# bwittmann/transoar

Hardware: AMD Instinct MI355X
Metric: training-step CT volumes/s, 160x160x256 Focused-Decoder (higher is better)
Workload: dtype bf16

## Files before the change

include/transoar_conv3d.h:

```cpp
#ifndef TRANSOAR_CONV3D_H
#define TRANSOAR_CONV3D_H

#include <stddef.h>
#include <stdint.h>

#ifdef __cplusplus
extern "C" {
#endif

enum {
  TRANSOAR_CONV_OK = 0,
  TRANSOAR_CONV_ERR_NULL = -1,
  TRANSOAR_CONV_ERR_DIM = -2,
  TRANSOAR_CONV_ERR_CHANNELS = -3
};

int transoar_conv3d_k3_forward(const void* x, const void* wk, const float* bias, void* y,
                               int N, int D, int H, int W, int Cin, int Cout, int stride,
                               int dilated_input, void* hip_stream);

int transoar_conv3d_k3_wgrad(const void* gyT, const void* xT3, float* dw, int N, int D, int H,
                             int W, int Cin, int Do, int Ho, int Wo, int Cout, int stride_dh,
                             void* hip_stream);

int transoar_conv3d_k3_forward_c1(const void* x, const void* wk, const float* bias, void* y, int N, int D, int H,
                                  int W, int Cout, void* hip_stream);

int transoar_conv3d_k3_stat_rows(int N, int D, int H, int W, int Cin, int Cout, int stride);
int transoar_conv3d_k3_forward_stats(const void* x, const void* wk, const float* bias, void* y, float* stat_part,
                                     int N, int D, int H, int W, int Cin, int Cout, void* hip_stream);

int transoar_conv3d_c1_forward(const void* x, const float* w, void* y, int N, int D, int H,
                               int W, int Cout, void* hip_stream);

int transoar_conv3d_k3_wgrad_lds(const void* x, const void* dy, float* partial, int n_wg, int N, int D,
                                 int H, int W, int Cin, int Cout, int ci0, int ci_n, int co0, int co_n,
                                 void* hip_stream);
int transoar_conv3d_k3_wgrad_tr(const void* x, const void* dy, float* partial, int n_wg, int N, int D,
                                 int H, int W, int Cin, int Cout, int ci0, int ci_n, int co0, int co_n,
                                 void* hip_stream);

int transoar_conv3d_c1_wgrad(const void* x, const void* dy, float* partial, int n_partial, int N, int D,
                             int H, int W, int Cout, void* hip_stream);
int transoar_conv3d_c1_wgrad_tr(const void* x, const void* dy, float* partial, int n_partial, int N, int D,
                                int H, int W, int Cout, void* hip_stream);

int transoar_layout_bf16(const void* in, void* out, int N, long V, int C, int to_channels_first,
                         void* hip_stream);

int transoar_conv3d_abi_version(void);

#ifdef __cplusplus
}
#endif
#endif
```

include/transoar_instnorm.h:

```cpp
#ifndef TRANSOAR_INSTNORM_H
#define TRANSOAR_INSTNORM_H

#ifdef __cplusplus
extern "C" {
#endif

enum {
  TRANSOAR_IN_OK = 0,
  TRANSOAR_IN_ERR_NULL = -1,
  TRANSOAR_IN_ERR_DIM = -2,
  TRANSOAR_IN_ERR_CHANNELS = -3
};

int transoar_instnorm_relu_forward(const void* x, const float* gamma, const float* beta, void* y,
                                   double* stats_ws, float* mean_rstd, int N, long V, int C,
                                   float eps, int relu, void* hip_stream);

int transoar_instnorm_relu_forward_parts(const void* x, const float* gamma, const float* beta, void* y,
                                         const float* stat_part, int rows_per_sample, double* stats_ws,
                                         float* mean_rstd, int N, long V, int C, float eps, int relu,
                                         void* hip_stream);

int transoar_instnorm_relu_backward(const void* x, const void* dy, const float* gamma,
                                    const float* beta, const float* mean_rstd, void* dx,
                                    double* red_ws, float* dparams, int N, long V, int C, int relu,
                                    void* hip_stream);

int transoar_instnorm_abi_version(void);

#ifdef __cplusplus
}
#endif
#endif
```

transoar_amd/backbone.py:

```python
import os

import torch
from torch import nn

from . import instnorm
from .conv3d import Conv3dK3, to_ncdhw
from .position_encoding import PositionEmbeddingLearned3D, PositionEmbeddingSine3D
from .swin_encoder import ConvPatchMerging, EncoderSwinBlock, PatchMerging
from .refine_block import DecoderDefAttnBlock
from .token_linear import token_linear


class EncoderCnnBlock(nn.Module):

    def __init__(self, in_channels, out_channels, kernel_size, stride, padding=1, bias=False,
                 affine=True, eps=1e-05):
        super().__init__()
        kernel_size, stride = tuple(kernel_size), tuple(stride)
        self._block = nn.Sequential(
            Conv3dK3(in_channels, out_channels, kernel_size, stride=stride, padding=padding, bias=bias),
            nn.InstanceNorm3d(out_channels, affine=affine, eps=eps),
            nn.ReLU(inplace=True),
            Conv3dK3(out_channels, out_channels, kernel_size, stride=1, padding=padding, bias=bias),
            nn.InstanceNorm3d(out_channels, affine=affine, eps=eps),
            nn.ReLU(inplace=True),
        )
        self._affine = affine

    fused_norm = True

    def _norm_relu(self, x, norm, part=None):
        if (EncoderCnnBlock.fused_norm and self._affine and x.dtype == torch.bfloat16
                and instnorm.supported(x, norm.num_features)):
            return instnorm.instance_norm_relu(x, norm.weight, norm.bias, norm.eps, relu=True, part=part)
        return torch.relu_(norm(x))

    def _conv_norm_relu(self, conv, norm, x):
        if (EncoderCnnBlock.fused_norm and self._affine and isinstance(conv, Conv3dK3) and norm.num_features <= 32):
            y, part = conv.forward_with_stats(x)
            if part is not None and not (y.dtype == torch.bfloat16 and instnorm.supported(y, norm.num_features)):
                part = None
            return self._norm_relu(y, norm, part)
        return self._norm_relu(conv(x), norm)

    def forward(self, x):
        if not x.is_cuda:
            return self._block(x)
        blk = self._block
        x = self._conv_norm_relu(blk[0], blk[1], x)
        return self._conv_norm_relu(blk[3], blk[4], x)


class Encoder(nn.Module):
    def __init__(self, config, debug=False):
        super().__init__()
        self._debug = debug
        self._stages = nn.ModuleList()
        cin, cout = config["in_channels"], config["start_channels"]
        swin = bool(config["use_encoder_attn"])
        depths = list(config["depths"])
        dpr = [float(v) for v in torch.linspace(0, config["drop_path_rate"], sum(depths))]
        merge = ConvPatchMerging if config["conv_merging"] else PatchMerging
        for stage_id, (kernel, stride) in enumerate(zip(config["conv_kernels"], config["strides"])):
            if swin and stage_id > 1:
                k = stage_id - 2
                stage = EncoderSwinBlock(
                    dim=cin, depth=depths[k], num_heads=config["num_heads"][k], window_size=config["window_size"],
                    mlp_ratio=config["mlp_ratio"], qkv_bias=config["qkv_bias"], qk_scale=config["qk_scale"],
                    drop=config["drop_rate"], attn_drop=config["attn_drop_rate"],
                    drop_path=dpr[sum(depths[:k]):sum(depths[:k + 1])], downsample=merge)
            else:
                stage = EncoderCnnBlock(cin, cout, kernel, stride)
# ... 134 lines not shown
```

transoar_amd/conv3d.py:

```python
import ctypes
import os

import torch
import torch.nn.functional as F
from torch import nn

from . import _native
from . import rows as _rows
from . import conv_gemm as _cg

_PKG = os.path.dirname(os.path.abspath(__file__))
_LIB_PATH = os.path.join(_PKG, "libtransoar_conv3d.so")
ABI_VERSION = 5


def _load():
    if not os.path.exists(_LIB_PATH):
        raise _native.NativeLibraryError("%s is not built (python transoar_amd/_build.py)" % _LIB_PATH)
    lib = ctypes.CDLL(_LIB_PATH)
    i, p = ctypes.c_int, ctypes.c_void_p
    lib.transoar_conv3d_k3_forward.restype = i
    lib.transoar_conv3d_k3_forward.argtypes = [p, p, p, p] + [i] * 8 + [p]
    lib.transoar_conv3d_k3_wgrad.restype = i
    lib.transoar_conv3d_k3_wgrad.argtypes = [p, p, p] + [i] * 10 + [p]
    lib.transoar_conv3d_k3_wgrad_lds.restype = i
    lib.transoar_conv3d_k3_wgrad_lds.argtypes = [p, p, p, i] + [i] * 10 + [p]
    lib.transoar_conv3d_k3_wgrad_tr.restype = i
    lib.transoar_conv3d_k3_wgrad_tr.argtypes = [p, p, p, i] + [i] * 10 + [p]
    lib.transoar_conv3d_c1_wgrad.restype = i
    lib.transoar_conv3d_c1_wgrad.argtypes = [p, p, p, i] + [i] * 5 + [p]
    lib.transoar_conv3d_c1_wgrad_tr.restype = i
    lib.transoar_conv3d_c1_wgrad_tr.argtypes = [p, p, p, i] + [i] * 5 + [p]
    lib.transoar_conv3d_k3_stat_rows.restype = i
    lib.transoar_conv3d_k3_stat_rows.argtypes = [i] * 7
    lib.transoar_conv3d_k3_forward_stats.restype = i
    lib.transoar_conv3d_k3_forward_stats.argtypes = [p, p, p, p, p] + [i] * 6 + [p]
    lib.transoar_conv3d_k3_forward_c1.restype = i
    lib.transoar_conv3d_k3_forward_c1.argtypes = [p, p, p, p] + [i] * 5 + [p]
    lib.transoar_conv3d_c1_forward.restype = i
    lib.transoar_conv3d_c1_forward.argtypes = [p, p, p] + [i] * 5 + [p]
    lib.transoar_layout_bf16.restype = i
    lib.transoar_layout_bf16.argtypes = [p, p, i, ctypes.c_long, i, i, p]
    lib.transoar_conv3d_abi_version.restype = i
    if lib.transoar_conv3d_abi_version() != ABI_VERSION:
        raise _native.NativeLibraryError("%s: ABI mismatch, rebuild" % _LIB_PATH)
    return lib


lib = _load()
CL3D = torch.channels_last_3d


def _check(rc, what):
    if rc != 0:
        raise RuntimeError("%s failed with code %d" % (what, rc))


def _stream():
    return torch.cuda.current_stream().cuda_stream


class _Relayout(torch.autograd.Function):

# ... 197 lines not shown
                wk, wkt = packs
            elif weight.requires_grad or x.requires_grad:
                wk, wkt = _cg.pack_both(weight)
            else:
                wk = _cg.pack_fwd(weight)
            y = _cg.conv_forward(xb, wk, bias.float() if bias is not None else None, stride)
        else:
            y = conv3d_k3_forward(xb, _pack_taps(weight), bias.float() if bias is not None else None, stride)
        ctx.save_for_backward(xb, weight, wkt)
        ctx.stride, ctx.has_bias = stride, bias is not None
        return (y, None) if want_stats else y

    @staticmethod
    def backward(ctx, gy, _gpart=None):
        xb, weight, wkt = ctx.saved_tensors
        gyb = _as_ndhwc(gy)
        gx = gw = gb = None
        need_x, need_w = ctx.needs_input_grad[0], ctx.needs_input_grad[1]
        ci, co = xb.shape[1], weight.shape[0]
        if need_x and _use_gemm(ci, co, ctx.stride):
            gx = _cg.conv_dgrad(gyb, wkt if wkt is not None else _cg.pack_dgrad(weight), ctx.stride, tuple(xb.shape[2:]))
        elif need_x:
            wt = weight.flip(2, 3, 4).permute(2, 3, 4, 1, 0).reshape(27, weight.shape[1], weight.shape[0])
            gx = conv3d_k3_forward(gyb, wt.to(torch.bfloat16).contiguous(), None, 1, dilated_input=ctx.stride == 2)
        if need_w:
            rows = gyb.numel() // gyb.shape[1]
            if ctx.stride == 1 and c1_wgrad_supported(xb, gyb):
                gw = conv3d_c1_wgrad(xb, gyb)
            elif ctx.stride == 1 and lds_wgrad_supported(xb, gyb) and (max(ci, co) <= 32 or rows >= (1 << 21)):
                gw = conv3d_k3_wgrad_lds(xb, gyb)
            elif ci % 8 == 0 and co % 8 == 0:
                gw = _cg.conv_wgrad(xb, gyb, ctx.stride)
            else:
                gw = conv3d_k3_wgrad(xb, gyb, ctx.stride)
            gw = gw.to(weight.dtype)
        if ctx.has_bias and ctx.needs_input_grad[2]:
            g2 = gyb.permute(0, 2, 3, 4, 1).reshape(-1, gyb.shape[1])
            gb = _rows.colsum_any(g2) if g2.is_contiguous() else gyb.float().sum(dim=(0, 2, 3, 4))
        return gx, gw, gb, None, None, None


def _use_gemm(cin, cout, stride):
    return cin >= 8 and cin % 8 == 0 and cout % 8 == 0 and (stride == 2 or cin > 24 or cout > 32)


def hip_conv_supported(x, conv):
    return (x.is_cuda and x.dtype == torch.bfloat16 and conv.kernel_size == (3, 3, 3) and conv.padding == (1, 1, 1)
            and conv.stride in ((1, 1, 1), (2, 2, 2)) and conv.dilation == (1, 1, 1) and conv.groups == 1
            and (conv.in_channels % 8 == 0
                 or (conv.in_channels == 1 and conv.stride == (1, 1, 1) and conv.out_channels <= 64))
            and conv.out_channels % 8 == 0 and (x.shape[-1] // conv.stride[0]) % 8 == 0
            and (conv.stride == (1, 1, 1) or all(s % 2 == 0 for s in x.shape[2:])))


class Conv3dK3(nn.Conv3d):
    enabled = True
    min_voxels = 0
    ndhwc_everywhere = os.environ.get("TRANSOAR_NDHWC_ALL", "1") == "1"
    _packs, _packs_version = None, -1

    def uses_gemm(self):
        return self.kernel_size == (3, 3, 3) and _use_gemm(self.in_channels, self.out_channels, self.stride[0])

    def forward(self, x):
# ... 22 lines not shown
```

transoar_amd/csrc/conv3d.hip:

```cpp
#include <hip/hip_runtime.h>
#include <algorithm>
#include <cstdlib>
#include <stdint.h>

#include "../../include/transoar_conv3d.h"

namespace transoar {

using bf16x8 = __attribute__((ext_vector_type(8))) __bf16;
using f32x16 = __attribute__((ext_vector_type(16))) float;
using u32x4c = __attribute__((ext_vector_type(4))) unsigned int;
using u32x2c = __attribute__((ext_vector_type(2))) unsigned int;

__device__ __forceinline__ unsigned short f2bf(float f) {
  return __builtin_bit_cast(unsigned short, static_cast<__bf16>(f));
}
__device__ __forceinline__ unsigned pack2_bf16(float a, float b) {
  typedef float f32x2_t __attribute__((ext_vector_type(2)));
  typedef __bf16 bf16x2_t __attribute__((ext_vector_type(2)));
  return __builtin_bit_cast(unsigned, __builtin_convertvector(f32x2_t{a, b}, bf16x2_t));
}
__device__ __forceinline__ float bf2f(unsigned short b) {
  return __uint_as_float(static_cast<unsigned int>(b) << 16);
}

constexpr unsigned kOOB = 0xfffffff0u;

struct ConvGeom {
// ... 593 lines not shown
        bp[j] = static_cast<unsigned>(bv[2 * j]) | (static_cast<unsigned>(bv[2 * j + 1]) << 16);
      }
      acc = __builtin_amdgcn_mfma_f32_32x32x16_bf16(__builtin_bit_cast(bf16x8, ap), __builtin_bit_cast(bf16x8, bp), acc,
                                                    0, 0, 0);
    }
  }
#pragma unroll
  for (int r = 0; r < 16; ++r) red[wave][r][lane] = acc[r];
  __syncthreads();
  if (wave == 0) {
    float* out = partial + static_cast<long>(blockIdx.x) * 1024;
#pragma unroll
    for (int r = 0; r < 16; ++r) {
      const float v = red[0][r][lane] + red[1][r][lane] + red[2][r][lane] + red[3][r][lane];
      out[((r & 3) + 8 * (r >> 2) + 4 * kg) * 32 + col] = v;
    }
  }
}

typedef short c1_s16x4 __attribute__((ext_vector_type(4)));
typedef short c1_s16x8 __attribute__((ext_vector_type(8)));
constexpr int kC1XP = 256 + 16;

template <int CO8>
__global__ __launch_bounds__(256) void conv3d_c1_wgrad_tr(const unsigned short* __restrict__ x, const unsigned short* __restrict__ dy,
                                                          float* __restrict__ partial, int N, int D, int H, int W, int Cout,
                                                          long n_rows, int rows_per_wg, unsigned x_bytes, unsigned dy_bytes) {
  __shared__ __attribute__((aligned(16))) unsigned char dyt[256 * 64 + 512];
  __shared__ __attribute__((aligned(16))) unsigned short xs[3][10][kC1XP];
  const int tid = threadIdx.x, lane = tid & 63, wave = tid >> 6;
  const int kg = lane >> 5;
  const __amdgpu_buffer_rsrc_t rx = __builtin_amdgcn_make_buffer_rsrc(const_cast<unsigned short*>(x), 0, static_cast<int>(x_bytes), 0x00020000);
  const __amdgpu_buffer_rsrc_t rdy = __builtin_amdgcn_make_buffer_rsrc(const_cast<unsigned short*>(dy), 0, static_cast<int>(dy_bytes), 0x00020000);
  for (int i = tid; i < (256 * 64 + 512) / 4; i += 256) reinterpret_cast<unsigned*>(dyt)[i] = 0u;
  for (int i = tid; i < 3 * 10 * kC1XP / 2; i += 256) reinterpret_cast<unsigned*>(&xs[0][0][0])[i] = 0u;

  f32x16 acc;
#pragma unroll
  for (int r = 0; r < 16; ++r) acc[r] = 0.f;
  const int t_row = 8 * kg + ((lane & 15) >> 2), t_ch = 16 * ((lane >> 4) & 1) + 4 * (lane & 3);
  const unsigned char* a_base = dyt + (64 * wave + t_row) * 64 + t_ch * 2;
  const int tap = lane & 31;
  const unsigned short* b_base = tap < 27 ? &xs[tap % 3][tap / 3][64 * wave + 8 * kg] : &xs[0][9][64 * wave + 8 * kg];
  typedef __attribute__((address_space(3))) c1_s16x4 lds_s16x4;

  const long row_beg = static_cast<long>(blockIdx.x) * rows_per_wg, row_end = min(n_rows, row_beg + rows_per_wg);
  u32x4c pdy[CO8], px[2];
  const int dy_pieces = W * CO8;
  auto prefetch = [&](long row) {
#pragma unroll
    for (int k = 0; k < CO8; ++k) {
      const int p = tid + 256 * k;
      pdy[k] = __builtin_amdgcn_raw_buffer_load_b128(rdy, p < dy_pieces ? static_cast<unsigned>(row) * static_cast<unsigned>(dy_pieces * 16) + p * 16 : 0x80000000u, 0, 0);
    }
    const int h = static_cast<int>(row % H);
    const long bd = row / H;
    const int d = static_cast<int>(bd % D);
#pragma unroll
    for (int k = 0; k < 2; ++k) {
      const int i = tid + 256 * k, r = i >> 5, piece = i & 31;
      const int id = d + r / 3 - 1, ih = h + r % 3 - 1;
      const bool ok = r < 9 && piece * 8 < W && static_cast<unsigned>(id) < static_cast<unsigned>(D) && static_cast<unsigned>(ih) < static_cast<unsigned>(H);
      px[k] = __builtin_amdgcn_raw_buffer_load_b128(rx, ok ? static_cast<unsigned>(((bd - d + id) * H + ih) * W + piece * 8) * 2u : 0x80000000u, 0, 0);
    }
  };
  if (row_beg < row_end) prefetch(row_beg);
  __syncthreads();
  for (long row = row_beg; row < row_end; ++row) {
#pragma unroll
    for (int k = 0; k < CO8; ++k) {
      const int p = tid + 256 * k;
      if (p < dy_pieces) *reinterpret_cast<u32x4c*>(dyt + (p / CO8) * 64 + (p % CO8) * 16) = pdy[k];
    }
#pragma unroll
    for (int k = 0; k < 2; ++k) {
      const int i = tid + 256 * k, r = i >> 5, piece = i & 31;
      const u32x4c v = px[k];
      unsigned left = __shfl_up(v[3], 1), right = __shfl_down(v[0], 1);
      if (piece == 0) left = 0u;
      if (piece * 8 + 8 >= W) right = 0u;
      if (r < 9 && piece * 8 < W) {
        u32x4c lo, hi;
        lo[0] = __builtin_amdgcn_alignbit(v[0], left, 16); lo[1] = __builtin_amdgcn_alignbit(v[1], v[0], 16);
        lo[2] = __builtin_amdgcn_alignbit(v[2], v[1], 16); lo[3] = __builtin_amdgcn_alignbit(v[3], v[2], 16);
        hi[0] = __builtin_amdgcn_alignbit(v[1], v[0], 16); hi[1] = __builtin_amdgcn_alignbit(v[2], v[1], 16);
        hi[2] = __builtin_amdgcn_alignbit(v[3], v[2], 16); hi[3] = __builtin_amdgcn_alignbit(right, v[3], 16);
        *reinterpret_cast<u32x4c*>(&xs[0][r][piece * 8]) = lo;
        *reinterpret_cast<u32x4c*>(&xs[1][r][piece * 8]) = v;
        *reinterpret_cast<u32x4c*>(&xs[2][r][piece * 8]) = hi;
      }
    }
    __syncthreads();
    if (row + 1 < row_end) prefetch(row + 1);
    if (64 * wave < W) {
#pragma unroll
// ... 273 lines not shown
extern "C" int transoar_conv3d_c1_wgrad_tr(const void* x, const void* dy, float* partial, int n_partial, int N, int D, int H,
                                           int W, int Cout, void* hip_stream) {
  if (!x || !dy || !partial) return TRANSOAR_CONV_ERR_NULL;
  if (N <= 0 || D <= 0 || H <= 0 || W <= 0 || Cout <= 0 || n_partial <= 0) return TRANSOAR_CONV_ERR_DIM;
  if (Cout > 32 || (Cout & 7) || (W & 63) || W > 256) return TRANSOAR_CONV_ERR_CHANNELS;
  const long n_rows = static_cast<long>(N) * D * H;
  const long xb = n_rows * W * 2, dyb = n_rows * W * Cout * 2;
  if (dyb >= 0x7ffffff0L) return TRANSOAR_CONV_ERR_DIM;
  const int rows_per_wg = static_cast<int>((n_rows + n_partial - 1) / n_partial);
#define TRANSOAR_C1TR(CO8)                                                                                                          \
  hipLaunchKernelGGL(conv3d_c1_wgrad_tr<CO8>, dim3(static_cast<unsigned>(n_partial)), dim3(256), 0, static_cast<hipStream_t>(hip_stream), \
                     static_cast<const unsigned short*>(x), static_cast<const unsigned short*>(dy), partial, N, D, H, W, Cout, n_rows,   \
                     rows_per_wg, static_cast<unsigned>(xb), static_cast<unsigned>(dyb))
  switch (Cout / 8) {
    case 1: TRANSOAR_C1TR(1); break;
    case 2: TRANSOAR_C1TR(2); break;
    case 3: TRANSOAR_C1TR(3); break;
    default: TRANSOAR_C1TR(4); break;
  }
#undef TRANSOAR_C1TR
  return static_cast<int>(hipGetLastError());
}

extern "C" int transoar_conv3d_c1_forward(const void* x, const float* w, void* y, int N, int D, int H, int W,
                                          int Cout, void* hip_stream) {
  if (!x || !w || !y) return TRANSOAR_CONV_ERR_NULL;
  if (N <= 0 || D <= 0 || H <= 0 || W <= 0 || Cout <= 0) return TRANSOAR_CONV_ERR_DIM;
  if ((Cout & 7) || Cout > transoar::kC1MaxCout) return TRANSOAR_CONV_ERR_CHANNELS;
  const long n_vox = static_cast<long>(N) * D * H * W;
  hipLaunchKernelGGL(conv3d_c1_fwd, dim3(static_cast<unsigned>((n_vox + 255) / 256)), dim3(256), 0,
                     static_cast<hipStream_t>(hip_stream), static_cast<const unsigned short*>(x), w,
                     static_cast<unsigned short*>(y), N, D, H, W, Cout, n_vox);
  return static_cast<int>(hipGetLastError());
}

extern "C" int transoar_layout_bf16(const void* in, void* out, int N, long V, int C, int to_channels_first,
                                    void* hip_stream) {
  if (!in || !out) return TRANSOAR_CONV_ERR_NULL;
  if (N <= 0 || V <= 0 || C <= 0) return TRANSOAR_CONV_ERR_DIM;
  if (C & 7) return TRANSOAR_CONV_ERR_CHANNELS;
  const dim3 grid(static_cast<unsigned>((V + 255) / 256), static_cast<unsigned>(N));
  hipStream_t st = static_cast<hipStream_t>(hip_stream);
  if (to_channels_first)
    hipLaunchKernelGGL(layout_vc_to_cv, grid, dim3(256), 0, st, static_cast<const unsigned short*>(in),
                       static_cast<unsigned short*>(out), V, C);
  else
    hipLaunchKernelGGL(layout_cv_to_vc, grid, dim3(256), 0, st, static_cast<const unsigned short*>(in),
                       static_cast<unsigned short*>(out), V, C);
  return static_cast<int>(hipGetLastError());
}

extern "C" int transoar_conv3d_abi_version(void) { return 5; }
```

transoar_amd/csrc/instnorm.hip:

```cpp
#include <hip/hip_runtime.h>
#include <stdint.h>

#include "../../include/transoar_instnorm.h"

namespace transoar {

using u32x4n = __attribute__((ext_vector_type(4))) unsigned int;
constexpr int kINThreads = 192;
constexpr int kINDepth = 4;
constexpr int kINBlocksPerCU = 4;
constexpr int kINDepthDx = 2;

__device__ __forceinline__ void unpack8(const u32x4n& r, float (&o)[8]) {
#pragma unroll
  for (int i = 0; i < 4; ++i) {
    o[2 * i] = __uint_as_float(r[i] << 16);
    o[2 * i + 1] = __uint_as_float(r[i] & 0xffff0000u);
  }
}
__device__ __forceinline__ unsigned short f2bf_n(float f) {
  return __builtin_bit_cast(unsigned short, static_cast<__bf16>(f));
}
__device__ __forceinline__ unsigned pack2_bf16_n(float a, float b) {
  typedef float f32x2_t __attribute__((ext_vector_type(2)));
  typedef __bf16 bf16x2_t __attribute__((ext_vector_type(2)));
  return __builtin_bit_cast(unsigned, __builtin_convertvector(f32x2_t{a, b}, bf16x2_t));
}
__device__ __forceinline__ u32x4n pack8(const float (&o)[8]) {
  u32x4n r;
#pragma unroll
  for (int i = 0; i < 4; ++i)
    r[i] = pack2_bf16_n(o[2 * i], o[2 * i + 1]);
  return r;
}

template <int K>
__device__ __forceinline__ void block_reduce_to_global(const float (&a)[K][8], int chunks, double* dst,
                                                       int dst_stride) {
  __shared__ float sm[kINThreads][K * 8 + 1];
  const int tid = threadIdx.x;
#pragma unroll
  for (int k = 0; k < K; ++k)
#pragma unroll
    for (int e = 0; e < 8; ++e) sm[tid][k * 8 + e] = a[k][e];
  __syncthreads();
  const int cols = chunks * K * 8;
  for (int c = tid; c < cols; c += kINThreads) {
    const int chunk = c / (K * 8), ke = c - chunk * (K * 8);
    double s = 0.0;
    for (int t = chunk; t < kINThreads; t += chunks) s += static_cast<double>(sm[t][ke]);
    const int k = ke >> 3, e = ke & 7;
    __hip_atomic_fetch_add(dst + static_cast<long>(chunk * 8 + e) * dst_stride + k, s, __ATOMIC_RELAXED,
                           __HIP_MEMORY_SCOPE_AGENT);
  }
}

__global__ __launch_bounds__(kINThreads) void instnorm_stats(const unsigned short* __restrict__ x,
// ... 144 lines not shown
    take(*reinterpret_cast<const u32x4n*>(x + base + v * C + chunk * 8), *reinterpret_cast<const u32x4n*>(dy + base + v * C + chunk * 8));
  block_reduce_to_global<2>(acc, chunks, red + static_cast<long>(n) * C * 2, 2);
}

__global__ __launch_bounds__(kINThreads) void instnorm_bwd_dx(
    const unsigned short* __restrict__ x, const unsigned short* __restrict__ dy,
    const float* __restrict__ mean_rstd, const float* __restrict__ gamma, const float* __restrict__ beta,
    const double* __restrict__ red, unsigned short* __restrict__ dx, long V, int C, int blocks_per_sample,
    int relu, float* __restrict__ dparams, int N) {
  const int chunks = C >> 3;
  const int n = blockIdx.x / blocks_per_sample, bi = blockIdx.x % blocks_per_sample;
  if (dparams && blockIdx.x == 0) {
    for (int i = threadIdx.x; i < 2 * C; i += kINThreads) {
      const int k = i / C, c = i - k * C;
      double s = 0.0;
      for (int nn = 0; nn < N; ++nn) s += red[(static_cast<long>(nn) * C + c) * 2 + k];
      dparams[i] = static_cast<float>(s);
    }
  }
  const int chunk = threadIdx.x % chunks;
  const long vstep = kINThreads / chunks;
  const long v_per_block = (V + blocks_per_sample - 1) / blocks_per_sample;
  const long v0 = bi * v_per_block, v1 = min(V, v0 + v_per_block);
  float m[8], rs[8], ga[8], be[8], mg[8], mgx[8];
#pragma unroll
  for (int e = 0; e < 8; ++e) {
    const int c = chunk * 8 + e;
    const long k = static_cast<long>(n) * C + c;
    m[e] = mean_rstd[k * 2];
    rs[e] = mean_rstd[k * 2 + 1];
    ga[e] = gamma[c];
    be[e] = beta[c];
    mg[e] = static_cast<float>(red[k * 2] / static_cast<double>(V));
    mgx[e] = static_cast<float>(red[k * 2 + 1] / static_cast<double>(V));
  }
  const long base = static_cast<long>(n) * V * C;
  auto put = [&](const u32x4n& px, const u32x4n& pg, long vv) {
    float f[8], g[8];
    unpack8(px, f);
    unpack8(pg, g);
#pragma unroll
    for (int e = 0; e < 8; ++e) {
      const float xh = (f[e] - m[e]) * rs[e];
      const float gg = (!relu || xh * ga[e] + be[e] > 0.f) ? g[e] : 0.f;
      f[e] = rs[e] * ga[e] * (gg - mg[e] - xh * mgx[e]);
    }
    *reinterpret_cast<u32x4n*>(dx + base + vv * C + chunk * 8) = pack8(f);
  };
  long v = v0 + threadIdx.x / chunks;
  for (; v + (kINDepthDx - 1) * vstep < v1; v += kINDepthDx * vstep) {
    u32x4n px[kINDepthDx], pg[kINDepthDx];
#pragma unroll
    for (int i = 0; i < kINDepthDx; ++i) {
      px[i] = *reinterpret_cast<const u32x4n*>(x + base + (v + i * vstep) * C + chunk * 8);
      pg[i] = *reinterpret_cast<const u32x4n*>(dy + base + (v + i * vstep) * C + chunk * 8);
    }
#pragma unroll
    for (int i = 0; i < kINDepthDx; ++i) put(px[i], pg[i], v + i * vstep);
  }
  for (; v < v1; v += vstep)
    put(*reinterpret_cast<const u32x4n*>(x + base + v * C + chunk * 8), *reinterpret_cast<const u32x4n*>(dy + base + v * C + chunk * 8), v);
}

static int pick_blocks(long V, int N, int C) {
  long per = (kINBlocksPerCU * 256L + N - 1) / N;
  const long cap = (V * (C >> 3) + 8L * kINThreads - 1) / (8L * kINThreads);
  if (per > cap) per = cap;
  return static_cast<int>(per < 1 ? 1 : per);
}

// ... 44 lines not shown
                     mean_rstd, V, C, eps, bps, relu);
  return static_cast<int>(hipGetLastError());
}

extern "C" int transoar_instnorm_relu_backward(const void* x, const void* dy, const float* gamma, const float* beta,
                                               const float* mean_rstd, void* dx, double* red_ws, float* dparams, int N, long V,
                                               int C, int relu, void* hip_stream) {
  const int rc = check(x, dy, N, V, C);
  if (rc) return rc;
  if (!gamma || !beta || !mean_rstd || !dx || !red_ws) return TRANSOAR_IN_ERR_NULL;
  hipStream_t st = static_cast<hipStream_t>(hip_stream);
  const int bps = pick_blocks(V, N, C);
  hipError_t e = hipMemsetAsync(red_ws, 0, sizeof(double) * 2 * N * C, st);
  if (e != hipSuccess) return static_cast<int>(e);
  hipLaunchKernelGGL(instnorm_bwd_reduce, dim3(N * bps), dim3(kINThreads), 0, st,
                     static_cast<const unsigned short*>(x), static_cast<const unsigned short*>(dy), mean_rstd, gamma,
                     beta, red_ws, V, C, bps, relu);
  hipLaunchKernelGGL(instnorm_bwd_dx, dim3(N * bps), dim3(kINThreads), 0, st, static_cast<const unsigned short*>(x),
                     static_cast<const unsigned short*>(dy), mean_rstd, gamma, beta, red_ws,
                     static_cast<unsigned short*>(dx), V, C, bps, relu, dparams, N);
  return static_cast<int>(hipGetLastError());
}

extern "C" int transoar_instnorm_abi_version(void) { return 3; }
```

transoar_amd/instnorm.py:

```python
import ctypes
import os

import torch

from . import _native
from .conv3d import to_ndhwc

_PKG = os.path.dirname(os.path.abspath(__file__))
_LIB_PATH = os.path.join(_PKG, "libtransoar_instnorm.so")


def _load():
    if not os.path.exists(_LIB_PATH):
        raise _native.NativeLibraryError("%s is not built (python transoar_amd/_build.py)" % _LIB_PATH)
    lib = ctypes.CDLL(_LIB_PATH)
    i, p, lg, f = ctypes.c_int, ctypes.c_void_p, ctypes.c_long, ctypes.c_float
    lib.transoar_instnorm_relu_forward.restype = i
    lib.transoar_instnorm_relu_forward.argtypes = [p, p, p, p, p, p, i, lg, i, f, i, p]
    lib.transoar_instnorm_relu_forward_parts.restype = i
    lib.transoar_instnorm_relu_forward_parts.argtypes = [p, p, p, p, p, i, p, p, i, lg, i, f, i, p]
    lib.transoar_instnorm_relu_backward.restype = i
    lib.transoar_instnorm_relu_backward.argtypes = [p, p, p, p, p, p, p, p, i, lg, i, i, p]
    lib.transoar_instnorm_abi_version.restype = i
    if lib.transoar_instnorm_abi_version() != 3:
        raise _native.NativeLibraryError("%s: ABI mismatch, rebuild" % _LIB_PATH)
    return lib


lib = _load()
CL3D = torch.channels_last_3d


def supported(x, channels):
    return (x.is_cuda and x.dtype == torch.bfloat16 and x.dim() == 5 and channels % 8 == 0
            and 192 % (channels // 8) == 0)


class _InstNormReLU(torch.autograd.Function):
    @staticmethod
    def forward(ctx, x, gamma, beta, eps, relu, part=None):
        x = to_ndhwc(x)
        n, c = x.shape[:2]
        v = x.shape[2] * x.shape[3] * x.shape[4]
        y = torch.empty_like(x, memory_format=CL3D)
        g32, b32 = gamma.float().contiguous(), beta.float().contiguous()
        ws = torch.empty((n, c, 2), dtype=torch.float64, device=x.device)
        mean_rstd = torch.empty((n, c, 2), dtype=torch.float32, device=x.device)
# ... 13 lines not shown
        ctx.relu, ctx.param_dtype = relu, gamma.dtype
        return y

    @staticmethod
    def backward(ctx, dy):
        x, g32, b32, mean_rstd = ctx.saved_tensors
        dy = to_ndhwc(dy)
        n, c = x.shape[:2]
        v = x.shape[2] * x.shape[3] * x.shape[4]
        dx = torch.empty_like(x, memory_format=CL3D)
        red = torch.empty((n, c, 2), dtype=torch.float64, device=x.device)
        with torch.cuda.device(x.device):
            dparams = torch.empty((2, c), dtype=torch.float32, device=x.device)
            rc = lib.transoar_instnorm_relu_backward(x.data_ptr(), dy.data_ptr(), g32.data_ptr(), b32.data_ptr(),
                                                     mean_rstd.data_ptr(), dx.data_ptr(), red.data_ptr(), dparams.data_ptr(), n, v, c,
                                                     1 if ctx.relu else 0, torch.cuda.current_stream().cuda_stream)
        if rc != 0:
            raise RuntimeError("transoar_instnorm_relu_backward failed with code %d" % rc)
        return dx, dparams[1].to(ctx.param_dtype), dparams[0].to(ctx.param_dtype), None, None, None


def instance_norm_relu(x, gamma, beta, eps=1e-5, relu=True, part=None):
    return _InstNormReLU.apply(x, gamma, beta, eps, relu, part)
```

Baseline: 64.13.

## Fuse stem conv instance-norm backward dx into the Cin=1 weight-gradient kernel

Adds a StemFused autograd path for the first encoder conv (Cin=1) plus its InstanceNorm+ReLU. In backward, the norm reduction runs once, and the norm's input-gradient is computed inside the c1 weight-gradient kernel as dy tiles are staged into LDS, so the full-size norm dx tensor is never written and reread. The input gradient is skipped because the stem input does not need one. Also shares the per-element dx helper through a header and pads the Cin=1 dgrad path. The cost is extra loads and coefficient math inside the wgrad kernel, plus changed launch bounds for that variant.

After: 64.75 (median of 6 runs). No clear change (+1.0%).

```diff
diff --git a/include/transoar_conv3d.h b/include/transoar_conv3d.h
--- a/include/transoar_conv3d.h
+++ b/include/transoar_conv3d.h
@@ -45,6 +45,11 @@
 int transoar_conv3d_c1_wgrad_tr(const void* x, const void* dy, float* partial, int n_partial, int N, int D,
                                 int H, int W, int Cout, void* hip_stream);
 
+int transoar_conv3d_c1_wgrad_tr_dx(const void* x, const void* x1, const void* dy, const float* mean_rstd,
+                                   const float* gamma, const float* beta, const double* red, float* dparams,
+                                   float* partial, int n_partial, int N, int D, int H, int W, int Cout,
+                                   void* hip_stream);
+
 int transoar_layout_bf16(const void* in, void* out, int N, long V, int C, int to_channels_first,
                          void* hip_stream);
 
diff --git a/include/transoar_instnorm.h b/include/transoar_instnorm.h
--- a/include/transoar_instnorm.h
+++ b/include/transoar_instnorm.h
@@ -26,6 +26,13 @@
                                     double* red_ws, float* dparams, int N, long V, int C, int relu,
                                     void* hip_stream);
 
+int transoar_instnorm_bwd_reduce(const void* x, const void* dy, const float* gamma, const float* beta,
+                                 const float* mean_rstd, double* red_ws, int N, long V, int C, int relu,
+                                 void* hip_stream);
+int transoar_instnorm_bwd_dx(const void* x, const void* dy, const float* gamma, const float* beta,
+                             const float* mean_rstd, const double* red, void* dx, float* dparams, int N, long V,
+                             int C, int relu, void* hip_stream);
+
 int transoar_instnorm_abi_version(void);
 
 #ifdef __cplusplus
diff --git a/transoar_amd/backbone.py b/transoar_amd/backbone.py
--- a/transoar_amd/backbone.py
+++ b/transoar_amd/backbone.py
@@ -4,7 +4,7 @@
 from torch import nn
 
 from . import instnorm
-from .conv3d import Conv3dK3, to_ncdhw
+from .conv3d import Conv3dK3, StemFused, stem_fused_supported, to_ncdhw
 from .position_encoding import PositionEmbeddingLearned3D, PositionEmbeddingSine3D
 from .swin_encoder import ConvPatchMerging, EncoderSwinBlock, PatchMerging
 from .refine_block import DecoderDefAttnBlock
@@ -43,11 +43,17 @@
             return self._norm_relu(y, norm, part)
         return self._norm_relu(conv(x), norm)
 
+    fused_stem = True
+
     def forward(self, x):
         if not x.is_cuda:
             return self._block(x)
         blk = self._block
-        x = self._conv_norm_relu(blk[0], blk[1], x)
+        if (EncoderCnnBlock.fused_stem and EncoderCnnBlock.fused_norm and self._affine and isinstance(blk[0], Conv3dK3)
+                and stem_fused_supported(x, blk[0])):
+            x = StemFused.apply(x, blk[0].weight, blk[1].weight, blk[1].bias, blk[1].eps)
+        else:
+            x = self._conv_norm_relu(blk[0], blk[1], x)
         return self._conv_norm_relu(blk[3], blk[4], x)
 
 
diff --git a/transoar_amd/conv3d.py b/transoar_amd/conv3d.py
--- a/transoar_amd/conv3d.py
+++ b/transoar_amd/conv3d.py
@@ -11,7 +11,7 @@
 
 _PKG = os.path.dirname(os.path.abspath(__file__))
 _LIB_PATH = os.path.join(_PKG, "libtransoar_conv3d.so")
-ABI_VERSION = 5
+ABI_VERSION = 6
 
 
 def _load():
@@ -39,6 +39,8 @@
     lib.transoar_conv3d_k3_forward_c1.argtypes = [p, p, p, p] + [i] * 5 + [p]
     lib.transoar_conv3d_c1_forward.restype = i
     lib.transoar_conv3d_c1_forward.argtypes = [p, p, p] + [i] * 5 + [p]
+    lib.transoar_conv3d_c1_wgrad_tr_dx.restype = i
+    lib.transoar_conv3d_c1_wgrad_tr_dx.argtypes = [p] * 9 + [i] * 6 + [p]
     lib.transoar_layout_bf16.restype = i
     lib.transoar_layout_bf16.argtypes = [p, p, i, ctypes.c_long, i, i, p]
     lib.transoar_conv3d_abi_version.restype = i
@@ -282,7 +284,10 @@
             gx = _cg.conv_dgrad(gyb, wkt if wkt is not None else _cg.pack_dgrad(weight), ctx.stride, tuple(xb.shape[2:]))
         elif need_x:
             wt = weight.flip(2, 3, 4).permute(2, 3, 4, 1, 0).reshape(27, weight.shape[1], weight.shape[0])
-            gx = conv3d_k3_forward(gyb, wt.to(torch.bfloat16).contiguous(), None, 1, dilated_input=ctx.stride == 2)
+            if ci == 1:
+                gx = conv3d_k3_forward(gyb, F.pad(wt, (0, 0, 0, 7)).to(torch.bfloat16).contiguous(), None, 1)[:, :1].contiguous()
+            else:
+                gx = conv3d_k3_forward(gyb, wt.to(torch.bfloat16).contiguous(), None, 1, dilated_input=ctx.stride == 2)
         if need_w:
             rows = gyb.numel() // gyb.shape[1]
             if ctx.stride == 1 and c1_wgrad_supported(xb, gyb):
@@ -300,6 +305,62 @@
         return gx, gw, gb, None, None, None
 
 
+
+def conv3d_c1_wgrad_dx(x, x1, gy, mean_rstd, g32, b32, red):
+    n, _, d, h, w = x.shape
+    co = gy.shape[1]
+    n_part = min(C1_WGRAD_TR_PARTIALS, n * d * h)
+    partial = torch.empty((n_part, 32, 32), dtype=torch.float32, device=x.device)
+    dparams = torch.empty((2, co), dtype=torch.float32, device=x.device)
+    with torch.cuda.device(x.device):
+        _check(lib.transoar_conv3d_c1_wgrad_tr_dx(x.data_ptr(), x1.data_ptr(), gy.data_ptr(), mean_rstd.data_ptr(), g32.data_ptr(),
+                                                  b32.data_ptr(), red.data_ptr(), dparams.data_ptr(), partial.data_ptr(), n_part,
+                                                  n, d, h, w, co, _stream()), "transoar_conv3d_c1_wgrad_tr_dx")
+    return _colsum(partial).view(32, 32)[:co, :27].reshape(co, 1, 3, 3, 3), dparams
+
+
+def stem_fused_supported(x, conv):
+    if not (Conv3dK3.enabled and Conv3dK3.stats_in_epilogue and C1_WGRAD_TR):
+        return False
+    if not (x.is_cuda and x.dim() == 5 and x.shape[1] == 1 and not (x.requires_grad and torch.is_grad_enabled())):
+        return False
+    amp = torch.is_autocast_enabled() and torch.get_autocast_gpu_dtype() == torch.bfloat16
+    if not (x.dtype == torch.bfloat16 or amp):
+        return False
+    c = conv.out_channels
+    if not (conv.in_channels == 1 and c % 8 == 0 and c <= 32 and 192 % (c // 8) == 0 and conv.bias is None
+            and conv.kernel_size == (3, 3, 3) and conv.padding == (1, 1, 1) and conv.stride == (1, 1, 1)
+            and conv.dilation == (1, 1, 1) and conv.groups == 1):
+        return False
+    n, _, d, h, w = x.shape
+    if w % 64 != 0 or w > 256:
+        return False
+    return lib.transoar_conv3d_k3_stat_rows(n, d, h, w, 1, c, 1) > 0
+
+
+class StemFused(torch.autograd.Function):
+
+    @staticmethod
+    def forward(ctx, x0, w1, gamma, beta, eps):
+        from . import instnorm as _in
+        x0b = x0.to(torch.bfloat16).contiguous()
+        g32, b32 = gamma.float().contiguous(), beta.float().contiguous()
+        x1, part1 = conv3d_k3_forward_stats(x0b, _pack_taps(F.pad(w1, (0, 0, 0, 0, 0, 0, 0, 7))), None)
+        y1, mean_rstd = _in.forward_parts(x1, g32, b32, eps, part1)
+        ctx.save_for_backward(x0b, x1, g32, b32, mean_rstd)
+        ctx.w_dtype, ctx.param_dtype = w1.dtype, gamma.dtype
+        return y1
+
+    @staticmethod
+    def backward(ctx, dy1):
+        from . import instnorm as _in
+        x0b, x1, g32, b32, mean_rstd = ctx.saved_tensors
+        dy1 = _as_ndhwc(dy1)
+        red = _in.bwd_reduce(x1, dy1, g32, b32, mean_rstd)
+        dw1, dparams = conv3d_c1_wgrad_dx(x0b, x1, dy1, mean_rstd, g32, b32, red)
+        return None, dw1.to(ctx.w_dtype), dparams[1].to(ctx.param_dtype), dparams[0].to(ctx.param_dtype), None
+
+
 def _use_gemm(cin, cout, stride):
     return cin >= 8 and cin % 8 == 0 and cout % 8 == 0 and (stride == 2 or cin > 24 or cout > 32)
 
diff --git a/transoar_amd/csrc/conv3d.hip b/transoar_amd/csrc/conv3d.hip
--- a/transoar_amd/csrc/conv3d.hip
+++ b/transoar_amd/csrc/conv3d.hip
@@ -4,6 +4,7 @@
 #include <stdint.h>
 
 #include "../../include/transoar_conv3d.h"
+#include "instnorm_elem.hpp"
 
 namespace transoar {
 
@@ -643,16 +644,40 @@
 typedef short c1_s16x8 __attribute__((ext_vector_type(8)));
 constexpr int kC1XP = 256 + 16;
 
-template <int CO8>
-__global__ __launch_bounds__(256) void conv3d_c1_wgrad_tr(const unsigned short* __restrict__ x, const unsigned short* __restrict__ dy,
+struct C1DxArgs {
+  const unsigned short* x1;
+  const float* mean_rstd;
+  const float* gamma;
+  const float* beta;
+  const double* red;
+  float* dparams;
+};
+
+template <int CO8, bool DX = false>
+__global__ __launch_bounds__(256, DX ? 4 : 1) void conv3d_c1_wgrad_tr(const unsigned short* __restrict__ x, const unsigned short* __restrict__ dy,
                                                           float* __restrict__ partial, int N, int D, int H, int W, int Cout,
-                                                          long n_rows, int rows_per_wg, unsigned x_bytes, unsigned dy_bytes) {
+                                                          long n_rows, int rows_per_wg, unsigned x_bytes, unsigned dy_bytes,
+                                                          C1DxArgs dxa = C1DxArgs{}) {
   __shared__ __attribute__((aligned(16))) unsigned char dyt[256 * 64 + 512];
   __shared__ __attribute__((aligned(16))) unsigned short xs[3][10][kC1XP];
   const int tid = threadIdx.x, lane = tid & 63, wave = tid >> 6;
   const int kg = lane >> 5;
   const __amdgpu_buffer_rsrc_t rx = __builtin_amdgcn_make_buffer_rsrc(const_cast<unsigned short*>(x), 0, static_cast<int>(x_bytes), 0x00020000);
   const __amdgpu_buffer_rsrc_t rdy = __builtin_amdgcn_make_buffer_rsrc(const_cast<unsigned short*>(dy), 0, static_cast<int>(dy_bytes), 0x00020000);
+  __shared__ __attribute__((aligned(16))) float coef[DX ? 7 : 1][DX ? 8 * CO8 : 1];
+  [[maybe_unused]] __amdgpu_buffer_rsrc_t rx1 = rdy;
+  [[maybe_unused]] int coef_n = -1;
+  if constexpr (DX) {
+    rx1 = __builtin_amdgcn_make_buffer_rsrc(const_cast<unsigned short*>(dxa.x1), 0, static_cast<int>(dy_bytes), 0x00020000);
+    if (dxa.dparams && blockIdx.x == 0) {
+      for (int i = tid; i < 2 * Cout; i += 256) {
+        const int k = i / Cout, c = i - k * Cout;
+        double sum = 0.0;
+        for (int nn = 0; nn < N; ++nn) sum += dxa.red[(static_cast<long>(nn) * Cout + c) * 2 + k];
+        dxa.dparams[i] = static_cast<float>(sum);
+      }
+    }
+  }
   for (int i = tid; i < (256 * 64 + 512) / 4; i += 256) reinterpret_cast<unsigned*>(dyt)[i] = 0u;
   for (int i = tid; i < 3 * 10 * kC1XP / 2; i += 256) reinterpret_cast<unsigned*>(&xs[0][0][0])[i] = 0u;
 
@@ -667,12 +692,15 @@
 
   const long row_beg = static_cast<long>(blockIdx.x) * rows_per_wg, row_end = min(n_rows, row_beg + rows_per_wg);
   u32x4c pdy[CO8], px[2];
+  [[maybe_unused]] u32x4c px1[DX ? CO8 : 1];
   const int dy_pieces = W * CO8;
   auto prefetch = [&](long row) {
 #pragma unroll
     for (int k = 0; k < CO8; ++k) {
       const int p = tid + 256 * k;
-      pdy[k] = __builtin_amdgcn_raw_buffer_load_b128(rdy, p < dy_pieces ? static_cast<unsigned>(row) * static_cast<unsigned>(dy_pieces * 16) + p * 16 : 0x80000000u, 0, 0);
+      const unsigned off = p < dy_pieces ? static_cast<unsigned>(row) * static_cast<unsigned>(dy_pieces * 16) + p * 16 : 0x80000000u;
+      pdy[k] = __builtin_amdgcn_raw_buffer_load_b128(rdy, off, 0, 0);
+      if constexpr (DX) px1[k] = __builtin_amdgcn_raw_buffer_load_b128(rx1, off, 0, 0);
     }
     const int h = static_cast<int>(row % H);
     const long bd = row / H;
@@ -688,10 +716,43 @@
   if (row_beg < row_end) prefetch(row_beg);
   __syncthreads();
   for (long row = row_beg; row < row_end; ++row) {
+    if constexpr (DX) {
+      const int n = static_cast<int>(row / (static_cast<long>(D) * H));
+      if (n != coef_n) {
+        coef_n = n;
+        if (tid < 8 * CO8) {
+          const long k = static_cast<long>(n) * Cout + tid;
+          const double V = static_cast<double>(static_cast<long>(D) * H * W);
+          const float rs = dxa.mean_rstd[k * 2 + 1], ga = dxa.gamma[tid];
+          coef[0][tid] = dxa.mean_rstd[k * 2];
+          coef[1][tid] = rs;
+          coef[2][tid] = ga;
+          coef[3][tid] = dxa.beta[tid];
+          coef[4][tid] = static_cast<float>(dxa.red[k * 2] / V);
+          coef[5][tid] = static_cast<float>(dxa.red[k * 2 + 1] / V);
+          coef[6][tid] = rs * ga;
+        }
+        __syncthreads();
+      }
+    }
 #pragma unroll
     for (int k = 0; k < CO8; ++k) {
       const int p = tid + 256 * k;
-      if (p < dy_pieces) *reinterpret_cast<u32x4c*>(dyt + (p / CO8) * 64 + (p % CO8) * 16) = pdy[k];
+      if (p < dy_pieces) {
+        u32x4c piece = pdy[k];
+        if constexpr (DX) {
+          const int c8 = (p % CO8) * 8;
+          float cf[7][8];
+#pragma unroll
+          for (int f = 0; f < 7; ++f) {
+            const float4 lo = *reinterpret_cast<const float4*>(&coef[f][c8]), hi = *reinterpret_cast<const float4*>(&coef[f][c8 + 4]);
+            cf[f][0] = lo.x; cf[f][1] = lo.y; cf[f][2] = lo.z; cf[f][3] = lo.w;
+            cf[f][4] = hi.x; cf[f][5] = hi.y; cf[f][6] = hi.z; cf[f][7] = hi.w;
+          }
+          piece = in_dx_piece(px1[k], pdy[k], cf[0], cf[1], cf[2], cf[3], cf[4], cf[5], cf[6], true);
+        }
+        *reinterpret_cast<u32x4c*>(dyt + (p / CO8) * 64 + (p % CO8) * 16) = piece;
+      }
     }
 #pragma unroll
     for (int k = 0; k < 2; ++k) {
@@ -1011,6 +1072,34 @@
   return static_cast<int>(hipGetLastError());
 }
 
+extern "C" int transoar_conv3d_c1_wgrad_tr_dx(const void* x, const void* x1, const void* dy, const float* mean_rstd,
+                                              const float* gamma, const float* beta, const double* red, float* dparams,
+                                              float* partial, int n_partial, int N, int D, int H, int W, int Cout,
+                                              void* hip_stream) {
+  if (!x || !x1 || !dy || !partial || !mean_rstd || !gamma || !beta || !red) return TRANSOAR_CONV_ERR_NULL;
+  if (N <= 0 || D <= 0 || H <= 0 || W <= 0 || Cout <= 0 || n_partial <= 0) return TRANSOAR_CONV_ERR_DIM;
+  if (Cout > 32 || (Cout & 7) || (W & 63) || W > 256) return TRANSOAR_CONV_ERR_CHANNELS;
+  const long n_rows = static_cast<long>(N) * D * H;
+  const long xb = n_rows * W * 2, dyb = n_rows * W * Cout * 2;
+  if (dyb >= 0x7ffffff0L) return TRANSOAR_CONV_ERR_DIM;
+  const int rows_per_wg = static_cast<int>((n_rows + n_partial - 1) / n_partial);
+  C1DxArgs a;
+  a.x1 = static_cast<const unsigned short*>(x1); a.mean_rstd = mean_rstd; a.gamma = gamma; a.beta = beta; a.red = red;
+  a.dparams = dparams;
+#define TRANSOAR_C1TR_DX(CO8)                                                                                                             \
+  hipLaunchKernelGGL((conv3d_c1_wgrad_tr<CO8, true>), dim3(static_cast<unsigned>(n_partial)), dim3(256), 0,                               \
+                     static_cast<hipStream_t>(hip_stream), static_cast<const unsigned short*>(x), static_cast<const unsigned short*>(dy), \
+                     partial, N, D, H, W, Cout, n_rows, rows_per_wg, static_cast<unsigned>(xb), static_cast<unsigned>(dyb), a)
+  switch (Cout / 8) {
+    case 1: TRANSOAR_C1TR_DX(1); break;
+    case 2: TRANSOAR_C1TR_DX(2); break;
+    case 3: TRANSOAR_C1TR_DX(3); break;
+    default: TRANSOAR_C1TR_DX(4); break;
+  }
+#undef TRANSOAR_C1TR_DX
+  return static_cast<int>(hipGetLastError());
+}
+
 extern "C" int transoar_conv3d_c1_forward(const void* x, const float* w, void* y, int N, int D, int H, int W,
                                           int Cout, void* hip_stream) {
   if (!x || !w || !y) return TRANSOAR_CONV_ERR_NULL;
@@ -1039,4 +1128,4 @@
   return static_cast<int>(hipGetLastError());
 }
 
-extern "C" int transoar_conv3d_abi_version(void) { return 5; }
+extern "C" int transoar_conv3d_abi_version(void) { return 6; }
diff --git a/transoar_amd/csrc/instnorm.hip b/transoar_amd/csrc/instnorm.hip
--- a/transoar_amd/csrc/instnorm.hip
+++ b/transoar_amd/csrc/instnorm.hip
@@ -2,37 +2,14 @@
 #include <stdint.h>
 
 #include "../../include/transoar_instnorm.h"
+#include "instnorm_elem.hpp"
 
 namespace transoar {
 
-using u32x4n = __attribute__((ext_vector_type(4))) unsigned int;
 constexpr int kINThreads = 192;
 constexpr int kINDepth = 4;
 constexpr int kINBlocksPerCU = 4;
 constexpr int kINDepthDx = 2;
-
-__device__ __forceinline__ void unpack8(const u32x4n& r, float (&o)[8]) {
-#pragma unroll
-  for (int i = 0; i < 4; ++i) {
-    o[2 * i] = __uint_as_float(r[i] << 16);
-    o[2 * i + 1] = __uint_as_float(r[i] & 0xffff0000u);
-  }
-}
-__device__ __forceinline__ unsigned short f2bf_n(float f) {
-  return __builtin_bit_cast(unsigned short, static_cast<__bf16>(f));
-}
-__device__ __forceinline__ unsigned pack2_bf16_n(float a, float b) {
-  typedef float f32x2_t __attribute__((ext_vector_type(2)));
-  typedef __bf16 bf16x2_t __attribute__((ext_vector_type(2)));
-  return __builtin_bit_cast(unsigned, __builtin_convertvector(f32x2_t{a, b}, bf16x2_t));
-}
-__device__ __forceinline__ u32x4n pack8(const float (&o)[8]) {
-  u32x4n r;
-#pragma unroll
-  for (int i = 0; i < 4; ++i)
-    r[i] = pack2_bf16_n(o[2 * i], o[2 * i + 1]);
-  return r;
-}
 
 template <int K>
 __device__ __forceinline__ void block_reduce_to_global(const float (&a)[K][8], int chunks, double* dst,
@@ -223,7 +200,7 @@
   const long vstep = kINThreads / chunks;
   const long v_per_block = (V + blocks_per_sample - 1) / blocks_per_sample;
   const long v0 = bi * v_per_block, v1 = min(V, v0 + v_per_block);
-  float m[8], rs[8], ga[8], be[8], mg[8], mgx[8];
+  float m[8], rs[8], ga[8], be[8], mg[8], mgx[8], rsga[8];
 #pragma unroll
   for (int e = 0; e < 8; ++e) {
     const int c = chunk * 8 + e;
@@ -234,19 +211,11 @@
     be[e] = beta[c];
     mg[e] = static_cast<float>(red[k * 2] / static_cast<double>(V));
     mgx[e] = static_cast<float>(red[k * 2 + 1] / static_cast<double>(V));
+    rsga[e] = rs[e] * ga[e];
   }
   const long base = static_cast<long>(n) * V * C;
   auto put = [&](const u32x4n& px, const u32x4n& pg, long vv) {
-    float f[8], g[8];
-    unpack8(px, f);
-    unpack8(pg, g);
-#pragma unroll
-    for (int e = 0; e < 8; ++e) {
-      const float xh = (f[e] - m[e]) * rs[e];
-      const float gg = (!relu || xh * ga[e] + be[e] > 0.f) ? g[e] : 0.f;
-      f[e] = rs[e] * ga[e] * (gg - mg[e] - xh * mgx[e]);
-    }
-    *reinterpret_cast<u32x4n*>(dx + base + vv * C + chunk * 8) = pack8(f);
+    *reinterpret_cast<u32x4n*>(dx + base + vv * C + chunk * 8) = in_dx_piece(px, pg, m, rs, ga, be, mg, mgx, rsga, relu != 0);
   };
   long v = v0 + threadIdx.x / chunks;
   for (; v + (kINDepthDx - 1) * vstep < v1; v += kINDepthDx * vstep) {
@@ -337,4 +306,32 @@
   return static_cast<int>(hipGetLastError());
 }
 
-extern "C" int transoar_instnorm_abi_version(void) { return 3; }
+extern "C" int transoar_instnorm_bwd_reduce(const void* x, const void* dy, const float* gamma, const float* beta,
+                                            const float* mean_rstd, double* red_ws, int N, long V, int C, int relu,
+                                            void* hip_stream) {
+  const int rc = check(x, dy, N, V, C);
+  if (rc) return rc;
+  if (!gamma || !beta || !mean_rstd || !red_ws) return TRANSOAR_IN_ERR_NULL;
+  hipStream_t st = static_cast<hipStream_t>(hip_stream);
+  const int bps = pick_blocks(V, N, C);
+  hipError_t e = hipMemsetAsync(red_ws, 0, sizeof(double) * 2 * N * C, st);
+  if (e != hipSuccess) return static_cast<int>(e);
+  hipLaunchKernelGGL(instnorm_bwd_reduce, dim3(N * bps), dim3(kINThreads), 0, st, static_cast<const unsigned short*>(x),
+                     static_cast<const unsigned short*>(dy), mean_rstd, gamma, beta, red_ws, V, C, bps, relu);
+  return static_cast<int>(hipGetLastError());
+}
+
+extern "C" int transoar_instnorm_bwd_dx(const void* x, const void* dy, const float* gamma, const float* beta,
+                                        const float* mean_rstd, const double* red, void* dx, float* dparams, int N, long V,
+                                        int C, int relu, void* hip_stream) {
+  const int rc = check(x, dy, N, V, C);
+  if (rc) return rc;
+  if (!gamma || !beta || !mean_rstd || !dx || !red) return TRANSOAR_IN_ERR_NULL;
+  const int bps = pick_blocks(V, N, C);
+  hipLaunchKernelGGL(instnorm_bwd_dx, dim3(N * bps), dim3(kINThreads), 0, static_cast<hipStream_t>(hip_stream),
+                     static_cast<const unsigned short*>(x), static_cast<const unsigned short*>(dy), mean_rstd, gamma, beta, red,
+                     static_cast<unsigned short*>(dx), V, C, bps, relu, dparams, N);
+  return static_cast<int>(hipGetLastError());
+}
+
+extern "C" int transoar_instnorm_abi_version(void) { return 4; }
diff --git a/transoar_amd/csrc/instnorm_elem.hpp b/transoar_amd/csrc/instnorm_elem.hpp
--- /dev/null
+++ b/transoar_amd/csrc/instnorm_elem.hpp
@@ -0,0 +1,68 @@
+#pragma once
+
+namespace transoar {
+
+using u32x4n = __attribute__((ext_vector_type(4))) unsigned int;
+
+__device__ __forceinline__ void unpack8(const u32x4n& r, float (&o)[8]) {
+#pragma unroll
+  for (int i = 0; i < 4; ++i) {
+    o[2 * i] = __uint_as_float(r[i] << 16);
+    o[2 * i + 1] = __uint_as_float(r[i] & 0xffff0000u);
+  }
+}
+__device__ __forceinline__ unsigned pack2_bf16_n(float a, float b) {
+  typedef float f32x2_t __attribute__((ext_vector_type(2)));
+  typedef __bf16 bf16x2_t __attribute__((ext_vector_type(2)));
+  return __builtin_bit_cast(unsigned, __builtin_convertvector(f32x2_t{a, b}, bf16x2_t));
+}
+__device__ __forceinline__ u32x4n pack8(const float (&o)[8]) {
+  u32x4n r;
+#pragma unroll
+  for (int i = 0; i < 4; ++i)
+    r[i] = pack2_bf16_n(o[2 * i], o[2 * i + 1]);
+  return r;
+}
+
+template <int E>
+__device__ __forceinline__ bool in_relu_open(float xh, float ga, float be) {
+#pragma clang fp contract(off)
+  if constexpr (E < 2) {
+    const float t = xh * ga;
+    return t + be > 0.f;
+  } else {
+    return __builtin_fmaf(xh, ga, be) > 0.f;
+  }
+}
+
+template <int E>
+__device__ __forceinline__ float in_dx(float x, float dy, float m, float rs, float ga, float be, float mg, float mgx,
+                                       float rsga, bool relu) {
+#pragma clang fp contract(off)
+  const float d = x - m;
+  const float xh = d * rs;
+  const float gg = (!relu || in_relu_open<E>(xh, ga, be)) ? dy : 0.f;
+  const float a = gg - mg;
+  return rsga * __builtin_fmaf(-xh, mgx, a);
+}
+
+template <int E = 0>
+__device__ __forceinline__ void in_dx8(const float (&f)[8], const float (&g)[8], const float (&m)[8], const float (&rs)[8],
+                                       const float (&ga)[8], const float (&be)[8], const float (&mg)[8],
+                                       const float (&mgx)[8], const float (&rsga)[8], bool relu, float (&o)[8]) {
+  if constexpr (E < 8) {
+    o[E] = in_dx<E>(f[E], g[E], m[E], rs[E], ga[E], be[E], mg[E], mgx[E], rsga[E], relu);
+    in_dx8<E + 1>(f, g, m, rs, ga, be, mg, mgx, rsga, relu, o);
+  }
+}
+__device__ __forceinline__ u32x4n in_dx_piece(const u32x4n& px, const u32x4n& pg, const float (&m)[8], const float (&rs)[8],
+                                              const float (&ga)[8], const float (&be)[8], const float (&mg)[8],
+                                              const float (&mgx)[8], const float (&rsga)[8], bool relu) {
+  float f[8], g[8], o[8];
+  unpack8(px, f);
+  unpack8(pg, g);
+  in_dx8(f, g, m, rs, ga, be, mg, mgx, rsga, relu, o);
+  return pack8(o);
+}
+
+}
diff --git a/transoar_amd/instnorm.py b/transoar_amd/instnorm.py
--- a/transoar_amd/instnorm.py
+++ b/transoar_amd/instnorm.py
@@ -8,6 +8,7 @@
 
 _PKG = os.path.dirname(os.path.abspath(__file__))
 _LIB_PATH = os.path.join(_PKG, "libtransoar_instnorm.so")
+ABI_VERSION = 4
 
 
 def _load():
@@ -21,8 +22,12 @@
     lib.transoar_instnorm_relu_forward_parts.argtypes = [p, p, p, p, p, i, p, p, i, lg, i, f, i, p]
     lib.transoar_instnorm_relu_backward.restype = i
     lib.transoar_instnorm_relu_backward.argtypes = [p, p, p, p, p, p, p, p, i, lg, i, i, p]
+    lib.transoar_instnorm_bwd_reduce.restype = i
+    lib.transoar_instnorm_bwd_reduce.argtypes = [p, p, p, p, p, p, i, lg, i, i, p]
+    lib.transoar_instnorm_bwd_dx.restype = i
+    lib.transoar_instnorm_bwd_dx.argtypes = [p, p, p, p, p, p, p, p, i, lg, i, i, p]
     lib.transoar_instnorm_abi_version.restype = i
-    if lib.transoar_instnorm_abi_version() != 3:
+    if lib.transoar_instnorm_abi_version() != ABI_VERSION:
         raise _native.NativeLibraryError("%s: ABI mismatch, rebuild" % _LIB_PATH)
     return lib
 
@@ -82,3 +87,47 @@
 
 def instance_norm_relu(x, gamma, beta, eps=1e-5, relu=True, part=None):
     return _InstNormReLU.apply(x, gamma, beta, eps, relu, part)
+
+
+
+def _nvc(x):
+    return x.shape[0], x.shape[2] * x.shape[3] * x.shape[4], x.shape[1]
+
+
+def _rc(rc, what):
+    if rc != 0:
+        raise RuntimeError("%s failed with code %d" % (what, rc))
+
+
+def forward_parts(x, g32, b32, eps, part, relu=True):
+    n, v, c = _nvc(x)
+    y = torch.empty_like(x, memory_format=CL3D)
+    ws = torch.empty((n, c, 2), dtype=torch.float64, device=x.device)
+    mean_rstd = torch.empty((n, c, 2), dtype=torch.float32, device=x.device)
+    with torch.cuda.device(x.device):
+        _rc(lib.transoar_instnorm_relu_forward_parts(x.data_ptr(), g32.data_ptr(), b32.data_ptr(), y.data_ptr(), part.data_ptr(),
+                                                     part.shape[0] // n, ws.data_ptr(), mean_rstd.data_ptr(), n, v, c, float(eps),
+                                                     1 if relu else 0, torch.cuda.current_stream().cuda_stream),
+            "transoar_instnorm_relu_forward_parts")
+    return y, mean_rstd
+
+
+def bwd_reduce(x, dy, g32, b32, mean_rstd, relu=True):
+    n, v, c = _nvc(x)
+    red = torch.empty((n, c, 2), dtype=torch.float64, device=x.device)
+    with torch.cuda.device(x.device):
+        _rc(lib.transoar_instnorm_bwd_reduce(x.data_ptr(), dy.data_ptr(), g32.data_ptr(), b32.data_ptr(), mean_rstd.data_ptr(),
+                                             red.data_ptr(), n, v, c, 1 if relu else 0,
+                                             torch.cuda.current_stream().cuda_stream), "transoar_instnorm_bwd_reduce")
+    return red
+
+
+def bwd_dx(x, dy, g32, b32, mean_rstd, red, relu=True):
+    n, v, c = _nvc(x)
+    dx = torch.empty_like(x, memory_format=CL3D)
+    dparams = torch.empty((2, c), dtype=torch.float32, device=x.device)
+    with torch.cuda.device(x.device):
+        _rc(lib.transoar_instnorm_bwd_dx(x.data_ptr(), dy.data_ptr(), g32.data_ptr(), b32.data_ptr(), mean_rstd.data_ptr(),
+                                         red.data_ptr(), dx.data_ptr(), dparams.data_ptr(), n, v, c, 1 if relu else 0,
+                                         torch.cuda.current_stream().cuda_stream), "transoar_instnorm_bwd_dx")
+    return dx, dparams
```
